# coderforlife/ms-compress

Hardware: AMD Instinct MI355X
Metric: input MB/s (lznt1 compress, bit-exact with the reference CPU encoder) (higher is better)
Workload: dtype u8; 1 GPU; BASELINE configs[4], lznt1: 16x replicated Silesia-shaped set: 192 files, one unit each (4 KiB chunks inside), 3391017280 B; units=192, bytes_rank0=3391017280, parallelism=shard-per-gpu x1, no data-path collective, lznt1_parity_checked=True

## Files before the change

ms_compress_amd/csrc/lznt1.hip:

```cpp
#include "common.h"
#include "kernels.h"

namespace msc {

#ifdef LZ_PROFILE
__device__ unsigned long long g_lz_prof[16];
#define LZ_T(i) { const unsigned long long t_ = __builtin_readcyclecounter(); t_acc[i] += t_ - t_prev; t_prev = t_; }
#define LZ_T0   unsigned long long t_prev = __builtin_readcyclecounter(); unsigned long long t_acc[16] = {0};
#define LZ_CNT(i, v) { t_acc[i] += (unsigned long long)(v); }
#define LZ_TEND if (lane == 0) { for (int i_ = 0; i_ < 16; ++i_) { atomicAdd(&g_lz_prof[i_], t_acc[i_]); } }
#else
#define LZ_T(i)
#define LZ_T0
#define LZ_CNT(i, v)
#define LZ_TEND
#endif

#ifdef LZ4_PROFILE_EVENTS
#define LZ4_PROFILE
#endif
#ifdef LZ4_PROFILE
#define LZ4_NSLOT 20
#define LZ4_NEV   (4 * LZ4_NSLOT)
#define LZ4_NPROF (LZ4_NEV + 4)
// ... 8 lines not shown
#define LZ_SELF     4u
#endif

__device__ __forceinline__ uint32_t lz_hash(uint32_t key24) { const uint32_t h = (key24 * 0x9E3779B1u) >> (32 - LZ_TBL_BITS); return h ? h : 1u; }

__device__ __forceinline__ uint32_t lz_shift(uint32_t pos)
{
	uint32_t z; asm("v_ffbh_u32 %0, %1" : "=v"(z) : "v"(pos - 1u));
	return (z - 16u) < 12u ? z - 16u : 12u;
}

__device__ __forceinline__ void     wst16(uint16_t* p, uint32_t v) { __hip_atomic_store(p, (uint16_t)v, __ATOMIC_RELAXED, __HIP_MEMORY_SCOPE_WAVEFRONT); }
__device__ __forceinline__ uint16_t wld16(uint16_t* p) { return __hip_atomic_load(p, __ATOMIC_RELAXED, __HIP_MEMORY_SCOPE_WAVEFRONT); }
__device__ __forceinline__ void     wst32(uint32_t* p, uint32_t v) { __hip_atomic_store(p, v, __ATOMIC_RELAXED, __HIP_MEMORY_SCOPE_WAVEFRONT); }
__device__ __forceinline__ uint32_t wld32(uint32_t* p) { return __hip_atomic_load(p, __ATOMIC_RELAXED, __HIP_MEMORY_SCOPE_WAVEFRONT); }
__device__ __forceinline__ void     wave_fence() { __builtin_amdgcn_fence(__ATOMIC_ACQ_REL, "wavefront", "local"); }

typedef uint16_t lz_u16x2 __attribute__((ext_vector_type(2)));
__device__ __forceinline__ uint32_t lz_entry32(uint16_t e) { lz_u16x2 v; v.x = e; return __builtin_bit_cast(uint32_t, v); }
__device__ __forceinline__ u64 lz_entry_below(uint32_t e, uint32_t p)
{
	u64 m; asm("v_cmp_gt_u32_sdwa %0, %1, %2 src0_sel:DWORD src1_sel:WORD_0" : "=s"(m) : "v"(p), "v"(e)); return m;
}
__device__ __forceinline__ uint4 lz_ld128(const uint8_t* base, uint32_t off)
{
	const uint32_t* a = reinterpret_cast<const uint32_t*>(base + (off & 0xFFCu));
	const uint32_t w0 = a[0], w1 = a[1], w2 = a[2], w3 = a[3], w4 = a[4];
	return make_uint4(alignbyte_addr(w1, w0, off), alignbyte_addr(w2, w1, off), alignbyte_addr(w3, w2, off), alignbyte_addr(w4, w3, off));
}
__device__ __forceinline__ uint32_t lz_ld32(const uint8_t* base, uint32_t off)
{
	const uint32_t* a = reinterpret_cast<const uint32_t*>(base + (off & 0xFFCu));
	return alignbyte_addr(a[1], a[0], off);
}
__device__ __forceinline__ uint32_t lz_lcp_tail(const uint8_t* d, uint32_t q, uint32_t p, uint32_t maxlen, uint32_t& it)
{
	uint32_t l = 16u;
	for (;;) {
		++it;
		uint4 a, b;
		a = lz_ld128(d, q + l); b = lz_ld128(d, p + l);
		const uint32_t f = first_nz_byte16(a.x ^ b.x, a.y ^ b.y, a.z ^ b.z, a.w ^ b.w);
		l += f;
		if (f < 16u || l >= maxlen) { break; }
	}
	return l;
}
__device__ __forceinline__ uint32_t lz_lcp_wave(const uint8_t* d, uint32_t q, uint32_t p, uint32_t l, uint32_t maxlen, uint32_t lane, uint32_t& steps)
{
	const uint32_t shq = q + l, shp = p + l;
	for (;;) {
		const uint32_t oq = q + l + 4u * lane, op = p + l + 4u * lane;
		const uint32_t* const aq = reinterpret_cast<const uint32_t*>(d + (oq & 0xFFCu));
		const uint32_t* const ap = reinterpret_cast<const uint32_t*>(d + (op & 0xFFCu));
		const uint32_t x = alignbyte_addr(aq[1], aq[0], shq) ^ alignbyte_addr(ap[1], ap[0], shp);
		const u64 ne = __builtin_amdgcn_ballot_w64(x != 0u);
		++steps;
		if (ne) {
			const uint32_t i = ctz64(ne);
			l += 4u * i + ((uint32_t)__builtin_ctz((uint32_t)__builtin_amdgcn_readlane((int)x, (int)i)) >> 3);
			break;
		}
		l += 256u;
		if (l >= maxlen) { break; }
	}
	return l < maxlen ? l : maxlen;
// ... 3 lines not shown
	const uint32_t a = ffbl_raw(x1) | 32u, b = ffbl_raw(x2) | 64u, c = ffbl_raw(x3) | 96u;
	return min3u(min3u(ffbl_raw(x0), a, b), c, capbits);
}
#define LZ_S1 8u
struct LzS1 { uint32_t x, y; };
__device__ __forceinline__ LzS1 lz_ld_s1(const uint8_t* base, uint32_t off)
{
	const uint32_t* a = reinterpret_cast<const uint32_t*>(base + (off & 0xFFCu));
	const uint32_t w0 = a[0], w1 = a[1], w2 = a[2];
	return LzS1{ alignbyte_addr(w1, w0, off), alignbyte_addr(w2, w1, off) };
}
__device__ __forceinline__ uint32_t lz_diff_bits_s1(uint32_t x0, uint32_t x1, uint32_t capbits)
{
	return min3u(ffbl_raw(x0), ffbl_raw(x1) | 32u, capbits);
}
struct LzS2 { uint32_t z, w; };
__device__ __forceinline__ LzS2 lz_ld_s2(const uint8_t* base, uint32_t off)
{
	const uint32_t* a = reinterpret_cast<const uint32_t*>(base + (off & 0xFFCu));
	const uint32_t w2 = a[2], w3 = a[3], w4 = a[4];
	return LzS2{ alignbyte_addr(w3, w2, off), alignbyte_addr(w4, w3, off) };
}
__device__ __forceinline__ uint32_t lz_diff_bits_s2(uint32_t xz, uint32_t xw, uint32_t capbits)
{
	return min3u(ffbl_raw(xz) | 64u, ffbl_raw(xw) | 96u, capbits);
}
__device__ __forceinline__ uint32_t lz_key(uint32_t bits, uint32_t q)
{
	uint32_t r; asm("v_bitop3_b32 %0, %1, %2, %3 bitop3:0x74" : "=v"(r) : "v"(bits << 9), "s"(0xFFFu), "v"(q)); return r;
}
__device__ __forceinline__ uint32_t lz_bit64(u64 m, uint32_t i) { u64 t; asm("s_lshr_b64 %0, %1, %2" : "=s"(t) : "s"(m), "s"(i) : "scc"); return (uint32_t)t & 1u; }
__device__ __forceinline__ uint32_t lz_need_bits(uint32_t len) { uint32_t r; asm("s_lshl3_add_u32 %0, %1, 8" : "=s"(r) : "s"(len) : "scc"); return r; }
struct LzWin { uint32_t key, o0, shift; u64 tokmask, matchmask; };
template <bool packed>
__device__ __forceinline__ uint32_t lz_window(const uint8_t* s_data, const void* tbl, const uint16_t* s_bucket, uint32_t n, uint32_t lane,
                                              uint32_t wbase, uint32_t entry, LzWin& r)
{
	entry = (uint32_t)__builtin_amdgcn_readfirstlane((int)entry); wbase = (uint32_t)__builtin_amdgcn_readfirstlane((int)wbase);
	const uint32_t wend = (wbase + 64u < n) ? wbase + 64u : n;
	const uint32_t p = wbase + lane;
	const LzS1 own = lz_ld_s1(s_data, p);
	const uint32_t o0 = own.x, o1 = own.y;
	const uint32_t shift = lz_shift(p);
	const uint32_t mask3 = (1u << shift) + 2u;
	uint32_t rel;
	asm("s_max_u32 %0, %1, %2\n\ts_sub_u32 %0, %0, %2" : "=&s"(rel) : "s"(entry), "s"(wbase) : "scc");
	const uint32_t lo = (wbase == 0 && rel == 0) ? 1u : rel;
	const uint32_t hi = n > wbase + 2u ? (n - wbase - 2u < 64u ? n - wbase - 2u : 64u) : 0u;
	const u64 act = sgpr64((~(u64)0 << lo) & (hi >= 64u ? ~(u64)0 : (((u64)1 << hi) - 1u)));
	const uint32_t maxlen = (n - p < mask3) ? n - p : mask3;
	uint32_t s;
	{
		const uint32_t h = lz_hash(o0 & 0xFFFFFFu);
		if (packed) {
			const uint32_t bit = h * 12u - 12u;
			const uint32_t* const t = static_cast<const uint32_t*>(tbl) + (bit >> 5);
			s = __builtin_amdgcn_alignbit(t[1], t[0], bit) & 0xFFFu;
		} else {
			s = static_cast<const uint16_t*>(tbl)[h - 1u];
		}
	}
	uint32_t key = 0;
	uint32_t q[LZ_SELF + 1u];
	u64 ex[LZ_SELF + 1u];
	#pragma unroll
	for (uint32_t j = 0; j <= LZ_SELF; ++j) { q[j] = lz_entry32(wld16(const_cast<uint16_t*>(s_bucket) + s + j)); }
	#pragma unroll
	for (uint32_t j = 0; j <= LZ_SELF; ++j) { ex[j] = (j ? ex[j - 1u] : act) & lz_entry_below(q[j], p); }
	const uint32_t capb = (maxlen < 16u ? maxlen : 16u) << 3, cap1 = (maxlen < LZ_S1 ? maxlen : LZ_S1) << 3;
	uint32_t kk[LZ_SELF];
	{
		uint32_t lb[LZ_SELF];
		{
			LzS1 c[LZ_SELF];
			#pragma unroll
			for (uint32_t k = 0; k < LZ_SELF; ++k) { c[k] = lz_ld_s1(s_data, q[k]); }
			#pragma unroll
			for (uint32_t k = 0; k < LZ_SELF; ++k) { lb[k] = lz_diff_bits_s1(c[k].x ^ o0, c[k].y ^ o1, cap1); }
		}
		u64 more = 0;
		#pragma unroll
		for (uint32_t k = 0; k < LZ_SELF; ++k) { more |= __builtin_amdgcn_ballot_w64(lb[k] >= 8u * LZ_S1) & ex[k]; }
		if (more & __builtin_amdgcn_ballot_w64(maxlen > LZ_S1)) {
			const LzS2 a = lz_ld_s2(s_data, p);
			LzS2 c[LZ_SELF];
			#pragma unroll
			for (uint32_t k = 0; k < LZ_SELF; ++k) { c[k] = lz_ld_s2(s_data, q[k]); }
			#pragma unroll
			for (uint32_t k = 0; k < LZ_SELF; ++k) {
				const uint32_t l2 = lz_diff_bits_s2(c[k].z ^ a.z, c[k].w ^ a.w, capb);
				lb[k] = lb[k] >= 8u * LZ_S1 ? l2 : lb[k];
			}
		}
		#pragma unroll
		for (uint32_t k = 0; k < LZ_SELF; ++k) {
			asm("v_cndmask_b32 %0, 0, %1, %2" : "=v"(kk[k]) : "v"(lz_key(lb[k], q[k])), "s"(ex[k]));
			key = kk[k] > key ? kk[k] : key;
		}
	}
	const u64 five = ex[LZ_SELF];
	u64 un = five & __builtin_amdgcn_ballot_w64(key < (maxlen << 12));
	const u64 lp = sgpr64(__builtin_amdgcn_ballot_w64(key >= (16u << 12)) & __builtin_amdgcn_ballot_w64(maxlen > 16u));
	u64 mm = __builtin_amdgcn_ballot_w64(key >= (3u << 12)) & ~un;
	u64 matchmask = 0;
	const uint32_t wn = (uint32_t)__builtin_amdgcn_readfirstlane((int)(wend - wbase));
	un = sgpr64(un); mm = sgpr64(mm);
	const u64 pend = sgpr64(un | lp);
	const uint32_t nx = lane + (key >> 12);
	const u64 restl = (un | mm) >> (nx & 63u);
	const uint32_t zl = min3u(ffbl_raw((uint32_t)restl), ffbl_raw((uint32_t)(restl >> 32)) | 32u, 64u);
	const uint32_t J = (nx + zl < wn) ? nx + zl : wn;
	uint32_t mp;
	{
		u64 rest; asm("s_lshr_b64 %0, %1, %2" : "=s"(rest) : "s"(un | mm), "s"(rel) : "scc");
		mp = rest ? rel + ctz64(rest) : wn;
	}
	if (mp < wn) do {
		asm volatile(
			"s_nop 3\n\t"
			"1:\n\t"
			"s_bitcmp1_b64 %[pend], %[mp]\n\t"
			"s_cbranch_scc1 3f\n\t"
			"s_bitset1_b64 %[mk], %[mp]\n\t"
			"v_readlane_b32 %[mp], %[J], %[mp]\n\t"
			"s_cmp_lt_u32 %[mp], %[wn]\n\t"
			"s_cbranch_scc1 1b\n\t"
			"3:\n\t"
			: [mp] "+s"(mp), [mk] "+s"(matchmask)
			: [pend] "s"(pend), [wn] "s"(wn), [J] "v"(J)
			: "scc");
		if (mp < wn) {
			const uint32_t sL = (uint32_t)__builtin_amdgcn_readlane((int)s, (int)mp);
			const uint32_t maxL = (uint32_t)__builtin_amdgcn_readlane((int)maxlen, (int)mp);
			const uint32_t pL = wbase + mp;
			uint32_t kbest = (uint32_t)__builtin_amdgcn_readlane((int)key, (int)mp);
			uint32_t fin = 1u;
			if (lz_bit64(lp, mp)) {
				const uint32_t qv = s_bucket[sL + lane % LZ_SELF];
				uint32_t nst = 0;
				#pragma unroll
				for (uint32_t k = 0; k < LZ_SELF; ++k) {
					if ((uint32_t)__builtin_amdgcn_readlane((int)kk[k], (int)mp) >> 16) {
						const uint32_t qk = (uint32_t)__builtin_amdgcn_readlane((int)qv, (int)k);
						const uint32_t l = lz_lcp_wave(s_data, qk, pL, 16u, maxL, lane, nst);
						const uint32_t kk = (l << 12) | (qk ^ 4095u);
						kbest = kk > kbest ? kk : kbest;
						if (l == maxL) { break; }
					}
				}
				fin = kbest < (maxL << 12) ? lz_bit64(un, mp) : 0u;
#ifdef LZ4_PROFILE_EVENTS
				if (lane == 0) { atomicAdd(&g_lz4_prof[LZ4_NEV + 2], 1ull); atomicAdd(&g_lz4_prof[LZ4_NEV + 3], (unsigned long long)nst); }
#endif
			}
			asm volatile("" : "+s"(fin));
			if (fin) {
				const uint32_t a0 = (uint32_t)__builtin_amdgcn_readlane((int)o0, (int)mp), a1 = (uint32_t)__builtin_amdgcn_readlane((int)o1, (int)mp);
#ifdef LZ4_PROFILE_EVENTS
				uint32_t nsteps = 0, ntail = 0;
#endif
				const uint32_t cap1L = (maxL < LZ_S1 ? maxL : LZ_S1) << 3;
				uint32_t need = kbest >> 12; need = lz_need_bits(need > 2u ? need : 2u);
				uint32_t base = sL + LZ_SELF;
// ... 31 lines not shown
				if (lane == 0) { atomicAdd(&g_lz4_prof[LZ4_NEV], (unsigned long long)nsteps); atomicAdd(&g_lz4_prof[LZ4_NEV + 1], (unsigned long long)ntail); }
#endif
			}
			{
				uint32_t t; u64 rs;
#pragma clang diagnostic push
#pragma clang diagnostic ignored "-Winline-asm"
				asm volatile(
					"s_bitset0_b64 %[un], %[mp]\n\t"
					"s_mov_b32 m0, %[mp]\n\t"
					"s_lshr_b32 %[t], %[kb], 12\n\t"
					"s_cmp_gt_u32 %[t], 2\n\t"
					"s_cselect_b32 %[t], %[t], 1\n\t"
					"s_cbranch_scc0 5f\n\t"
					"s_bitset1_b64 %[mk], %[mp]\n\t"
					"5:\n\t"
					"v_writelane_b32 %[key], %[kb], m0\n\t"
					"s_add_u32 %[mp], %[mp], %[t]\n\t"
					"s_or_b64 %[rs], %[un], %[mm]\n\t"
					"s_lshr_b64 %[rs], %[rs], %[mp]\n\t"
					"s_ff1_i32_b64 %[t], %[rs]\n\t"
					"s_min_u32 %[t], %[t], 64\n\t"
					"s_add_u32 %[mp], %[mp], %[t]\n\t"
					: [un] "+s"(un), [mk] "+s"(matchmask), [mp] "+s"(mp), [key] "+v"(key), [t] "=&s"(t), [rs] "=&s"(rs)
					: [kb] "s"(kbest), [mm] "s"(mm)
					: "scc", "m0");
#pragma clang diagnostic pop
			}
		}
	} while (mp < wn);
	matchmask = sgpr64(matchmask);
	uint32_t mend; asm("v_cndmask_b32 %0, 0, %1, %2" : "=v"(mend) : "v"(p + (key >> 12)), "s"(matchmask));
	const uint32_t reach = wave_incl_scan_max(mend);
	const u64 range = (~(u64)0 << rel) & (wn >= 64u ? ~(u64)0 : (((u64)1 << wn) - 1u));
	const u64 tokmask = range & (matchmask | __builtin_amdgcn_ballot_w64(reach <= p));
	const uint32_t wreach = (uint32_t)__builtin_amdgcn_readlane((int)reach, 63);
	const uint32_t cur = wreach > wend ? wreach : wend;

	r.key = key; r.o0 = o0; r.shift = shift; r.tokmask = tokmask; r.matchmask = matchmask;
	return cur;
}

template <bool serial>
__device__ __forceinline__ uint32_t lz_ordered_add(uint32_t* addr, uint32_t v, bool active, uint32_t lane)
{
	uint32_t old = 0;
	if (!serial) { if (active) { old = __hip_atomic_fetch_add(addr, v, __ATOMIC_RELAXED, __HIP_MEMORY_SCOPE_WAVEFRONT); } }
	else { for (uint32_t l = 0; l < 64u; ++l) { if (lane == l && active) { old = __hip_atomic_fetch_add(addr, v, __ATOMIC_RELAXED, __HIP_MEMORY_SCOPE_WAVEFRONT); } wave_fence(); } }
	return old;
}

template <bool serial, bool DEV = false>
__global__ __launch_bounds__(64) void lznt1_chunk_kernel(const uint8_t* __restrict__ d_in, BatchTables bt,
                                                        uint8_t* __restrict__ slots, uint32_t* __restrict__ slot_size)
{
	struct __attribute__((aligned(16))) Lds {
		uint8_t  data[4096 + 32];
		uint16_t bucket[4096];
		uint16_t cnt[LZ_TBL];
		uint32_t flagacc[16];
		uint32_t flagpos[16];
	};
	__shared__ Lds L;
	uint8_t* const s_data = L.data; uint16_t* const s_cnt = L.cnt; uint16_t* const s_bucket = L.bucket;
	uint32_t* const s_flagacc = L.flagacc; uint32_t* const s_flagpos = L.flagpos;

	const uint32_t lane = threadIdx.x;
// ... 134 lines not shown
extern "C" void mscomp_amd_debug_lz_prof(unsigned long long* out, int reset)
{
	(void)hipMemcpyFromSymbol(out, HIP_SYMBOL(g_lz_prof), sizeof(unsigned long long) * 16);
	if (reset) { unsigned long long z[16] = {0}; (void)hipMemcpyToSymbol(HIP_SYMBOL(g_lz_prof), z, sizeof z); }
}
#endif

#define LZ4_NSEG 4u
#ifndef LZ4_B1
#define LZ4_B1 21u
#define LZ4_B2 38u
#define LZ4_B3 52u
#endif
__device__ __forceinline__ uint32_t lz4_seg_start(uint32_t j) { return j == 0 ? 0u : j == 1 ? LZ4_B1 : j == 2 ? LZ4_B2 : j == 3 ? LZ4_B3 : 64u; }
#ifndef LZ4_P1
#define LZ4_P1 15u
#define LZ4_P2 39u
#endif
__host__ __device__ constexpr uint32_t lz4_max3(uint32_t a, uint32_t b, uint32_t c) { return a > b ? (a > c ? a : c) : (b > c ? b : c); }
__host__ __device__ constexpr uint32_t lz4_field_bits(uint32_t batches) { return batches * 64u <= 0x3FFu ? 10u : 11u; }
#define LZ4_PMAX lz4_max3(LZ4_P1, LZ4_P2 - LZ4_P1, 64u - LZ4_P2)
#define LZ4_F0 lz4_field_bits(LZ4_P1)
#define LZ4_F1 lz4_field_bits(LZ4_P2 - LZ4_P1)
#define LZ4_F2 lz4_field_bits(64u - LZ4_P2)
static_assert(LZ4_P1 >= 1u && LZ4_P1 < LZ4_P2 && LZ4_P2 < 64u, "three parts, none empty");
static_assert(LZ4_P1 * 64u <= (1u << LZ4_F0) - 1u && (LZ4_P2 - LZ4_P1) * 64u <= (1u << LZ4_F1) - 1u && (64u - LZ4_P2) * 64u <= (1u << LZ4_F2) - 1u, "a part fits its count field");
static_assert(LZ4_F0 + LZ4_F1 + LZ4_F2 <= 32u, "the three fields share a dword");
static_assert(LZ4_P1 <= LZ4_PMAX && LZ4_P2 - LZ4_P1 <= LZ4_PMAX && 64u - LZ4_P2 <= LZ4_PMAX, "LZ4_PMAX");
#define LZ4_MAXM 22u
#ifdef LZ4_PROFILE
extern "C" void mscomp_amd_debug_lz4_prof(unsigned long long* out) { (void)hipMemcpyFromSymbol(out, HIP_SYMBOL(g_lz4_prof), sizeof(unsigned long long) * LZ4_NPROF); unsigned long long z[LZ4_NPROF] = {0}; (void)hipMemcpyToSymbol(HIP_SYMBOL(g_lz4_prof), z, sizeof z); }
#endif
static_assert(LZNT1_REC == 2u * 64u * LZ4_MAXM * sizeof(uint16_t), "kernels.h: LZNT1_REC = two areas of 64 windows of match tokens");
template <bool serial, bool DEV = false>
__global__ __launch_bounds__(256) void lznt1_chunk4_kernel(const uint8_t* __restrict__ d_in, BatchTables bt,
                                                          uint8_t* __restrict__ slots, uint32_t* __restrict__ slot_size, uint16_t* __restrict__ recs)
{
	struct Ctl {
		u64      tok[64], mat[64];
		uint16_t endc[64];
		uint32_t prog[LZ4_NSEG];
		uint32_t used[LZ4_NSEG];
		uint32_t segctr;
		uint32_t total[2];
		uint8_t  rep[64];
	};
	struct __attribute__((aligned(16))) Lds {
		uint8_t  data[4096];
		uint16_t bucket[4096];
		union {
			uint16_t cnt[LZ_TBL];
			struct { uint32_t ends[LZ_TBL * 12u / 32u]; Ctl ctl; } parse;
		} t;
	};
	static_assert(LZ_TBL == 4096u, "the pack below hands 16 bucket ends to each of 256 threads");
	static_assert(sizeof(Lds) <= 20480, "eight blocks per CU");
	static_assert(offsetof(Lds, t) == offsetof(Lds, bucket) + sizeof(Lds::bucket) && sizeof(Lds::bucket) + sizeof(Lds::t) == LZ_TBL * sizeof(uint32_t),
	              "the sort's count words (one dword per bucket) lie over the bucket array and the union behind it");
	__shared__ Lds L;
	uint32_t* const s_cw = reinterpret_cast<uint32_t*>(L.bucket);
	uint8_t* const s_data = L.data; uint16_t* const s_cnt = L.t.cnt; uint16_t* const s_bucket = L.bucket;
	Ctl& C = L.t.parse.ctl;
	u64* const s_tok = C.tok; u64* const s_mat = C.mat; uint16_t* const s_endc = C.endc; uint8_t* const s_rep = C.rep;
	uint32_t* const s_prog = C.prog; uint32_t* const s_used = C.used; uint32_t& s_segctr = C.segctr; uint32_t* const s_total = C.total;
	uint16_t* const s_T = s_cnt;
	uint16_t* const s_S = s_cnt + 64;
	uint16_t* const s_flagpos = s_cnt + 128;
	uint32_t* const s_flagacc = reinterpret_cast<uint32_t*>(s_cnt + 640);

	const uint32_t tid = threadIdx.x, lane = tid & 63u;
	uint32_t c, wv;
	c = blockIdx.x; wv = (uint32_t)__builtin_amdgcn_readfirstlane((int)(tid >> 6));
	if (DEV && past_real_chunks(bt, c)) { if (tid == 0) { slot_size[c] = 0; } return; }
	uint32_t park = 0;
#define LZ4_PARK(i, v) { park = lane == (i) ? (uint32_t)(v) : park; }
#define LZ4_FETCH(i) ({ asm volatile("" : "+v"(park)); (uint32_t)__builtin_amdgcn_readlane((int)park, (int)(i)); })
	LZ4_PARK(0, (uintptr_t)slots) LZ4_PARK(1, (uintptr_t)slots >> 32) LZ4_PARK(2, (uintptr_t)slot_size) LZ4_PARK(3, (uintptr_t)slot_size >> 32)
	LZ4_PARK(4, c) LZ4_PARK(5, wv)
	asm volatile("" : "+v"(park));
	const uint32_t u = unit_of_chunk(bt.chunk_prefix, bt.n_units, c);
	const u64 coff = (u64)(c - bt.chunk_prefix[u]) * 4096u;
	const u64 left = bt.in_len[u] - coff;
	const uint32_t n = left < 4096u ? (uint32_t)left : 4096u;
	const uint8_t* __restrict__ src = d_in + bt.in_off[u] + coff;
	uint16_t* __restrict__ rec = recs + (u64)c * (LZNT1_REC / sizeof(uint16_t));

#ifdef LZ4_PROFILE
	uint32_t z_prev; asm volatile("v_mov_b32 %0, %1" : "=v"(z_prev) : "s"((uint32_t)__builtin_readcyclecounter()));
	uint32_t z_acc = 0;
#define LZ4_T(i) { uint32_t t_; asm volatile("v_mov_b32 %0, %1" : "=v"(t_) : "s"((uint32_t)__builtin_readcyclecounter())); z_acc += lane == (i) ? t_ - z_prev : 0u; z_prev = t_; }
#define LZ4_TEND { if (lane < LZ4_NSLOT) { atomicAdd(&g_lz4_prof[LZ4_NSLOT * wv + lane], (unsigned long long)z_acc); } }
#else
#define LZ4_T(i)
#define LZ4_TEND
#endif
	{
		const uint32_t nvec = (((uintptr_t)src & 15u) == 0) ? (n & ~15u) : 0u;
		for (uint32_t i = tid * 16u; i < nvec; i += 4096u) { *reinterpret_cast<uint4*>(s_data + i) = *reinterpret_cast<const uint4*>(src + i); }
		for (uint32_t i = nvec + tid; i < n; i += 256u) { s_data[i] = src[i]; }
		for (uint32_t i = n + tid; i < 4096u; i += 256u) { s_data[i] = 0; }
		for (uint32_t i = tid * 4u; i < LZ_TBL; i += 1024u) { *reinterpret_cast<uint4*>(s_cw + i) = make_uint4(0, 0, 0, 0); }
	}
	LZ4_T(0)
	__syncthreads();
	LZ4_T(1)
	{
		const uint32_t nb = (n + 63u) >> 6;
		const uint32_t pb0 = wv == 0 ? 0u : wv == 1u ? LZ4_P1 : wv == 2u ? LZ4_P2 : 64u;
		const uint32_t pe = wv == 0 ? LZ4_P1 : wv == 1u ? LZ4_P2 : 64u;
		const uint32_t pb1 = pe < nb ? pe : nb;
		const uint32_t fsh = wv == 0 ? 0u : wv == 1u ? LZ4_F0 : LZ4_F0 + LZ4_F1;
		const uint32_t fm = (1u << (wv == 0 ? LZ4_F0 : wv == 1u ? LZ4_F1 : LZ4_F2)) - 1u;
		uint32_t hr[LZ4_PMAX];
		#pragma unroll
		for (uint32_t i = 0; i < LZ4_PMAX; ++i) { hr[i] = 0; }
		#pragma unroll
		for (uint32_t j0 = 0; j0 < LZ4_PMAX; j0 += 8u) {
			if (pb0 + j0 < pb1) {
				uint32_t h[8], old[8];
				#pragma unroll
				for (uint32_t j = 0; j < 8u; ++j) { if (j0 + j < LZ4_PMAX) { h[j] = lz_hash(lz_ld32(s_data, (pb0 + j0 + j) * 64u + lane) & 0xFFFFFFu); } }
				#pragma unroll
				for (uint32_t j = 0; j < 8u; ++j) {
					if (j0 + j < LZ4_PMAX) { const uint32_t b = pb0 + j0 + j; old[j] = lz_ordered_add<serial>(s_cw + h[j], 1u << fsh, b < pb1 && b * 64u + lane + 2u < n, lane); }
				}
				#pragma unroll
				for (uint32_t j = 0; j < 8u; ++j) { if (j0 + j < LZ4_PMAX) { hr[j0 + j] = (h[j] << 12) | ((old[j] >> fsh) & fm); } }
			}
		}
		LZ4_T(2)
		__syncthreads();
		LZ4_T(3)
		static_assert(LZ4_P2 * 64u < 4096u, "rank + counts in front stay in 12 bits");
		if (wv == 1u || wv == 2u) {
			const uint32_t m1 = wv == 2u ? (1u << LZ4_F1) - 1u : 0u;
			#pragma unroll
			for (uint32_t j0 = 0; j0 < LZ4_PMAX; j0 += 8u) {
				if (pb0 + j0 < pb1) {
					uint32_t w[8];
					#pragma unroll
					for (uint32_t j = 0; j < 8u; ++j) { if (j0 + j < LZ4_PMAX) { w[j] = s_cw[hr[j0 + j] >> 12]; } }
					#pragma unroll
					for (uint32_t j = 0; j < 8u; ++j) { if (j0 + j < LZ4_PMAX) { hr[j0 + j] += (w[j] & ((1u << LZ4_F0) - 1u)) + ((w[j] >> LZ4_F0) & m1); } }
					__builtin_amdgcn_sched_barrier(0);
				}
			}
		}
		uint32_t tot[8], sum = 0;
		#pragma unroll
		for (uint32_t k = 0; k < 4u; ++k) {
			const uint4 a = reinterpret_cast<const uint4*>(s_cw)[4u * tid + k];
			uint32_t x[4] = { a.x, a.y, a.z, a.w };
			#pragma unroll
			for (uint32_t i = 0; i < 4u; ++i) { x[i] = (x[i] & ((1u << LZ4_F0) - 1u)) + ((x[i] >> LZ4_F0) & ((1u << LZ4_F1) - 1u)) + (x[i] >> (LZ4_F0 + LZ4_F1)); }
			if (k == 0 && tid == 0) { x[0] = 0; }
			sum += (x[0] + x[1]) + (x[2] + x[3]);
			tot[2u * k] = x[0] | (x[1] << 16); tot[2u * k + 1u] = x[2] | (x[3] << 16);
// ... 13 lines not shown
			uint32_t* const o = L.t.parse.ends + 6u * tid;
			#pragma unroll
			for (int k = 0; k < 2; ++k) {
				uint32_t v[8];
				#pragma unroll
				for (int i = 0; i < 4; ++i) { r += tot[4 * k + i] & 0xFFFFu; v[2 * i] = r; r += tot[4 * k + i] >> 16; v[2 * i + 1] = r; }
				o[3 * k]      = v[0] | (v[1] << 12) | (v[2] << 24);
				o[3 * k + 1u] = (v[2] >> 8) | (v[3] << 4) | (v[4] << 16) | (v[5] << 28);
				o[3 * k + 2u] = (v[5] >> 4) | (v[6] << 8) | (v[7] << 20);
			}
			if (tid < LZ4_NSEG) { s_prog[tid] = 0; s_used[tid] = 0; }
			if (tid < 16u) { reinterpret_cast<uint32_t*>(s_rep)[tid] = 0; }
			if (tid == 0) { s_segctr = 0; }
		}
		LZ4_T(6)
		__syncthreads();
		LZ4_T(7)
		#pragma unroll
		for (uint32_t j0 = 0; j0 < LZ4_PMAX; j0 += 8u) {
			if (pb0 + j0 < pb1) {
				uint32_t st[8];
				#pragma unroll
				for (uint32_t j = 0; j < 8u; ++j) {
					if (j0 + j < LZ4_PMAX) {
						const uint32_t bit = (hr[j0 + j] >> 12) * 12u - 12u;
						const uint32_t* const t = L.t.parse.ends + (bit >> 5);
						st[j] = __builtin_amdgcn_alignbit(t[1], t[0], bit) & 0xFFFu;
					}
				}
				#pragma unroll
				for (uint32_t j = 0; j < 8u; ++j) {
					if (j0 + j < LZ4_PMAX) {
						const uint32_t b = pb0 + j0 + j, p = b * 64u + lane;
						if (b < pb1 && p + 2u < n) { s_bucket[st[j] + (hr[j0 + j] & 0xFFFu)] = (uint16_t)p; }
					}
				}
			}
		}
	}
	LZ4_T(8)
	__syncthreads();
	const uint32_t* const tbl = L.t.parse.ends;
	LZ4_T(9)

	const uint32_t nw = (n + 63u) >> 6;
#define LZ4_WINDOW(w_, entry_, cur_out, a_) { \
		const uint32_t wb_ = (w_) * 64u; const uint32_t we_ = (wb_ + 64u < n) ? wb_ + 64u : n; \
		if ((entry_) >= we_) { if (lane == 0) { s_tok[w_] = 0; s_mat[w_] = 0; } cur_out = (entry_); } \
		else { \
			LzWin r_; cur_out = lz_window<true>(s_data, tbl, s_bucket, n, lane, wb_, (entry_), r_); \
			if (__builtin_amdgcn_inverse_ballot_w64(r_.matchmask)) { \
				const uint32_t p_ = wb_ + lane, best_ = r_.key >> 12; \
				uint16_t* __restrict__ const recw_ = rec + ((a_) * 64u + (w_)) * LZ4_MAXM; \
				recw_[popc_below(r_.matchmask)] = (uint16_t)(((p_ - (4095u - (r_.key & 0xFFFu)) - 1u) << r_.shift) | (best_ - 3u)); \
			} \
			if (lane == 0) { s_tok[w_] = r_.tokmask; s_mat[w_] = r_.matchmask; } \
		} \
		if ((a_) && lane == 0) { s_rep[w_] = 1; } }
#define LZ4_UNI(x) ((uint32_t)__builtin_amdgcn_readfirstlane((int)(x)))
	for (;;) {
		uint32_t seg = 0;
		if (lane == 0) { seg = atomicAdd(&s_segctr, 1u); }
		seg = (uint32_t)__builtin_amdgcn_readfirstlane((int)seg);
		const uint32_t a0 = lz4_seg_start(seg);
		if (a0 >= nw) { break; }
		const uint32_t a1 = (lz4_seg_start(seg + 1u) < nw) ? lz4_seg_start(seg + 1u) : nw;
		uint32_t entry = a0 * 64u;
		for (uint32_t w = a0; w < a1; w = LZ4_UNI(w + 1u)) {
			uint32_t cur;
			LZ4_WINDOW(w, entry, cur, 0u)
			entry = LZ4_UNI(cur);
			if (lane == 0) { s_endc[w] = (uint16_t)cur; }
			wave_fence();
			if (lane == 0) { __hip_atomic_store(&s_prog[seg], w + 1u, __ATOMIC_RELAXED, __HIP_MEMORY_SCOPE_WORKGROUP); }
		}
		if (a1 < nw) {
			if (lane == 0) { s_used[seg + 1u] = entry; }
			if (entry != a1 * 64u) {
				const uint32_t wlim = (lz4_seg_start(seg + 2u) < nw) ? lz4_seg_start(seg + 2u) : nw;
				for (uint32_t w = a1; w < wlim; w = LZ4_UNI(w + 1u)) {
					while (LZ4_UNI(__hip_atomic_load(&s_prog[seg + 1u], __ATOMIC_RELAXED, __HIP_MEMORY_SCOPE_WORKGROUP)) <= w) { __builtin_amdgcn_s_sleep(2); }
					wave_fence();
					const uint32_t spec = LZ4_UNI(s_endc[w]);
					uint32_t cur;
					LZ4_WINDOW(w, entry, cur, 1u)
					entry = LZ4_UNI(cur);
// ... 13 lines not shown
			if (e2 == LZ4_UNI(s_used[j])) { continue; }
			uint32_t wl = lz4_seg_start(j);
			for (uint32_t w = lz4_seg_start(j); w < nw; w = LZ4_UNI(w + 1u)) {
				const uint32_t spec = LZ4_UNI(s_endc[w]);
				uint32_t cur;
				LZ4_WINDOW(w, e2, cur, 1u)
				e2 = LZ4_UNI(cur);
				if (lane == 0) { s_endc[w] = (uint16_t)cur; }
				wave_fence();
				wl = w + 1u;
				if (cur == spec) { break; }
			}
			if (lane == 0) { for (uint32_t jj = j + 1u; jj < LZ4_NSEG && lz4_seg_start(jj) < wl; ++jj) { s_used[jj] = s_endc[lz4_seg_start(jj) - 1u]; } }
			wave_fence();
		}
	}
	LZ4_T(12)
	__syncthreads();
	LZ4_T(13)
	for (uint32_t i = tid; i < 512u; i += 256u) { s_flagacc[i] = 0; }
	wv = LZ4_FETCH(5); c = LZ4_FETCH(4);
	const uint32_t w0 = wv * 16u, w1 = (w0 + 16u < nw) ? w0 + 16u : nw;
	typedef __attribute__((address_space(1))) uint8_t  g_u8;
	typedef __attribute__((address_space(1))) uint32_t g_u32;
	g_u8* __restrict__ const img = (g_u8*)((uintptr_t)LZ4_FETCH(0) | ((uintptr_t)LZ4_FETCH(1) << 32)) + (u64)c * LZNT1_SLOT;
	g_u32* __restrict__ const szp = (g_u32*)((uintptr_t)LZ4_FETCH(2) | ((uintptr_t)LZ4_FETCH(3) << 32)) + c;
	static_assert(LZNT1_SLOT <= 0xFFFFFFFFu && (LZ4_MAXM & 1u) == 0 && LZ4_NSEG * 16u * LZ4_MAXM <= 4096u, "a window's tokens are whole dwords; four pieces fit the bucket array");
	uint32_t* const s_ptk = reinterpret_cast<uint32_t*>(s_bucket) + wv * (16u * LZ4_MAXM / 2u);
	const uint32_t wl0 = w0 + (lane & 15u);
	const u64 tokv = wl0 < w1 ? s_tok[wl0] : (u64)0, matv = wl0 < w1 ? s_mat[wl0] : (u64)0;
#ifndef LZ4_PROBE_EMIT
	{
		const uint32_t info = wl0 < w1 ? (uint32_t)__popcll(matv) | ((uint32_t)s_rep[wl0] << 8) : 0u;
		const uint32_t* __restrict__ const rec32 = reinterpret_cast<const uint32_t*>(rec);
		uint32_t v[3]; bool ld[3];
		#pragma unroll
		for (uint32_t k = 0; k < 3u; ++k) {
			const uint32_t idx = lane + 64u * k, wl = idx / (LZ4_MAXM / 2u), m2 = idx - wl * (LZ4_MAXM / 2u);
			const uint32_t inf = (uint32_t)__builtin_amdgcn_ds_bpermute((int)(wl * 4u), (int)info);
			ld[k] = idx < 16u * LZ4_MAXM / 2u && 2u * m2 < (inf & 0xFFu);
			v[k] = ld[k] ? rec32[((inf >> 8) * 64u + w0 + wl) * (LZ4_MAXM / 2u) + m2] : 0u;
		}
		#pragma unroll
		for (uint32_t k = 0; k < 3u; ++k) { if (ld[k]) { s_ptk[lane + 64u * k] = v[k]; } }
	}
#endif
	if (wv == 0) {
		const u64 tm = lane < nw ? s_tok[lane] : (u64)0, mk = lane < nw ? s_mat[lane] : (u64)0;
		const uint32_t nt = (uint32_t)__popcll(tm), ns = nt + (uint32_t)__popcll(mk);
		const uint32_t ti = wave_incl_scan_add_u32(nt), si = wave_incl_scan_add_u32(ns);
		s_T[lane] = (uint16_t)(ti - nt); s_S[lane] = (uint16_t)(si - ns);
		if (lane == 63u) { s_total[0] = ti; s_total[1] = si; }
	}
	LZ4_T(14)
	__syncthreads();
	LZ4_T(15)
	const uint32_t T = s_total[0], S = s_total[1];
	const uint32_t csize = ((T + 7u) >> 3) + S;
	uint32_t total;
	if (csize < n) {
		const uint32_t tsv = (uint32_t)s_T[wl0] | ((uint32_t)s_S[wl0] << 16);
		const uint32_t nwin = LZ4_UNI(w1 > w0 ? w1 - w0 : 0u);
		#pragma unroll 1
		for (uint32_t k = 0; k < nwin; ++k) {
			const u64 tokmask = ((u64)(uint32_t)__builtin_amdgcn_readlane((int)(uint32_t)(tokv >> 32), (int)k) << 32) | (uint32_t)__builtin_amdgcn_readlane((int)(uint32_t)tokv, (int)k);
			if (tokmask == 0) { continue; }
			const u64 matchmask = ((u64)(uint32_t)__builtin_amdgcn_readlane((int)(uint32_t)(matv >> 32), (int)k) << 32) | (uint32_t)__builtin_amdgcn_readlane((int)(uint32_t)matv, (int)k);
// ... 6 lines not shown
				const uint32_t lit = s_data[(w0 + k) * 64u + lane];
#ifdef LZ4_PROBE_EMIT
				const uint16_t tok = 0x1003u;
#else
				const uint16_t tok = reinterpret_cast<const uint16_t*>(s_ptk)[k * LZ4_MAXM + mbl];
#endif
				uint32_t lo; asm("v_cndmask_b32 %0, %1, %2, %3" : "=v"(lo) : "v"(lit), "v"(lz_entry32(tok)), "s"(matchmask));
				img[pos] = (uint8_t)lo;
				if (__builtin_amdgcn_inverse_ballot_w64(matchmask)) {
					uint32_t p1 = pos; asm("" : "+v"(p1));
					(img + p1)[1] = (uint8_t)(tok >> 8);
					atomicOr(&s_flagacc[t >> 3], 1u << (t & 7u));
				}
			}
		}
		LZ4_T(16)
		__syncthreads();
		LZ4_T(17)
		#pragma unroll 1
		for (uint32_t g = tid; g < ((T + 7u) >> 3); g += 256u) { uint32_t fp = s_flagpos[g]; asm("" : "+v"(fp)); img[fp] = (uint8_t)s_flagacc[g]; }
		if (tid == 0) { img[0] = (uint8_t)(0xB000u | (csize - 1u)); img[1] = (uint8_t)((0xB000u | (csize - 1u)) >> 8); }
		total = 2u + csize;
	} else {
		const uint32_t hdr = 0x3000u | (n - 1u);
		for (uint32_t k = tid; k < (n + 2u + 3u) / 4u; k += 256u) {
			uint32_t o = 4u * k; asm("" : "+v"(o));
			*(g_u32*)(img + o) = (k == 0) ? (hdr | (ld16(s_data) << 16)) : ld32(s_data + 4u * k - 2u);
		}
		total = 2u + n;
	}
	if (tid == 0) { *szp = total; }
	LZ4_T(18)
	LZ4_TEND
#undef LZ4_WINDOW
#undef LZ4_UNI
#undef LZ4_PARK
#undef LZ4_FETCH
}

template <bool DEV>
static void launch_lznt1_chunks_t(hipStream_t st, const uint8_t* d_in, const BatchTables& bt, uint8_t* slots, uint32_t* slot_size, uint16_t* recs,
                                  int mode, bool serial)
{
	if (mode == 1) {
		if (serial) { hipLaunchKernelGGL((lznt1_chunk_kernel<true, DEV>), dim3(bt.n_chunks), dim3(64), 0, st, d_in, bt, slots, slot_size); }
		else { hipLaunchKernelGGL((lznt1_chunk_kernel<false, DEV>), dim3(bt.n_chunks), dim3(64), 0, st, d_in, bt, slots, slot_size); }
	} else {
		if (serial) { hipLaunchKernelGGL((lznt1_chunk4_kernel<true, DEV>), dim3(bt.n_chunks), dim3(256), 0, st, d_in, bt, slots, slot_size, recs); }
		else { hipLaunchKernelGGL((lznt1_chunk4_kernel<false, DEV>), dim3(bt.n_chunks), dim3(256), 0, st, d_in, bt, slots, slot_size, recs); }
	}
}
void launch_lznt1_chunks_dev(hipStream_t st, const uint8_t* d_in, const BatchTables& bt, uint8_t* slots, uint32_t* slot_size, uint16_t* recs,
                             int mode, bool serial);
#ifndef LZNT1_DEV_TU
static int g_lznt1_mode = 0;
void set_lznt1_mode(int mode) { g_lznt1_mode = mode; }
void launch_lznt1_chunks(hipStream_t st, const uint8_t* d_in, const BatchTables& bt, uint8_t* slots, uint32_t* slot_size, uint16_t* recs, bool dev)
{
	if (bt.n_chunks == 0) { return; }
	const int mode = g_lznt1_mode ? g_lznt1_mode : 2;
	const bool serial = serial_atomics_on_current_device();
	if (dev) { launch_lznt1_chunks_dev(st, d_in, bt, slots, slot_size, recs, mode, serial); }
	else { launch_lznt1_chunks_t<false>(st, d_in, bt, slots, slot_size, recs, mode, serial); }
}
#else
void launch_lznt1_chunks_dev(hipStream_t st, const uint8_t* d_in, const BatchTables& bt, uint8_t* slots, uint32_t* slot_size, uint16_t* recs,
                             int mode, bool serial)
{
// ... 6 lines not shown
```

Measured before the change: 88850 MB/s.

## Specialize LZNT1 chunk kernel body for full 4 KiB chunks

Splits the chunk4 kernel into a templated body that is instantiated twice, once for full 4096-byte chunks and once for any length, and picks between them at runtime. In the full-chunk version, window bounds, active masks, the walk-loop limit and the hash-insert predicates become compile-time constants, and a lane-based aligned load replaces the general unaligned load. The aim is to cut scalar bookkeeping and branches in the hot window loop for nearly all chunks. In exchange the code is larger, which risks instruction-cache pressure and higher register use.

```diff
diff --git a/ms_compress_amd/csrc/lznt1.hip b/ms_compress_amd/csrc/lznt1.hip
--- a/ms_compress_amd/csrc/lznt1.hip
+++ b/ms_compress_amd/csrc/lznt1.hip
@@ -64,6 +64,11 @@
 {
 	const uint32_t* a = reinterpret_cast<const uint32_t*>(base + (off & 0xFFCu));
 	return alignbyte_addr(a[1], a[0], off);
+}
+__device__ __forceinline__ uint32_t lz_ld32_lane(const uint8_t* a4, uint32_t lane)
+{
+	const uint32_t* a = reinterpret_cast<const uint32_t*>(a4);
+	return alignbyte_addr(a[1], a[0], lane);
 }
 __device__ __forceinline__ uint32_t lz_lcp_tail(const uint8_t* d, uint32_t q, uint32_t p, uint32_t maxlen, uint32_t& it)
 {
@@ -133,12 +138,13 @@
 __device__ __forceinline__ uint32_t lz_bit64(u64 m, uint32_t i) { u64 t; asm("s_lshr_b64 %0, %1, %2" : "=s"(t) : "s"(m), "s"(i) : "scc"); return (uint32_t)t & 1u; }
 __device__ __forceinline__ uint32_t lz_need_bits(uint32_t len) { uint32_t r; asm("s_lshl3_add_u32 %0, %1, 8" : "=s"(r) : "s"(len) : "scc"); return r; }
 struct LzWin { uint32_t key, o0, shift; u64 tokmask, matchmask; };
-template <bool packed>
+template <bool packed, bool FULL = false>
 __device__ __forceinline__ uint32_t lz_window(const uint8_t* s_data, const void* tbl, const uint16_t* s_bucket, uint32_t n, uint32_t lane,
                                               uint32_t wbase, uint32_t entry, LzWin& r)
 {
+	if (FULL) { n = 4096u; }
 	entry = (uint32_t)__builtin_amdgcn_readfirstlane((int)entry); wbase = (uint32_t)__builtin_amdgcn_readfirstlane((int)wbase);
-	const uint32_t wend = (wbase + 64u < n) ? wbase + 64u : n;
+	const uint32_t wend = FULL ? wbase + 64u : ((wbase + 64u < n) ? wbase + 64u : n);
 	const uint32_t p = wbase + lane;
 	const LzS1 own = lz_ld_s1(s_data, p);
 	const uint32_t o0 = own.x, o1 = own.y;
@@ -146,9 +152,18 @@
 	const uint32_t mask3 = (1u << shift) + 2u;
 	uint32_t rel;
 	asm("s_max_u32 %0, %1, %2\n\ts_sub_u32 %0, %0, %2" : "=&s"(rel) : "s"(entry), "s"(wbase) : "scc");
-	const uint32_t lo = (wbase == 0 && rel == 0) ? 1u : rel;
-	const uint32_t hi = n > wbase + 2u ? (n - wbase - 2u < 64u ? n - wbase - 2u : 64u) : 0u;
-	const u64 act = sgpr64((~(u64)0 << lo) & (hi >= 64u ? ~(u64)0 : (((u64)1 << hi) - 1u)));
+	u64 act;
+	if (FULL) {
+		uint32_t lo;
+		asm("s_or_b32 %0, %1, %2\n\ts_cselect_b32 %0, %2, 1" : "=&s"(lo) : "s"(wbase), "s"(rel) : "scc");
+		const uint32_t top = wbase == 4032u ? 0x3FFFFFFFu : 0xFFFFFFFFu;
+		const u64 m = ~(u64)0 << lo;
+		act = sgpr64(((u64)((uint32_t)(m >> 32) & top) << 32) | (uint32_t)m);
+	} else {
+		const uint32_t lo = (wbase == 0 && rel == 0) ? 1u : rel;
+		const uint32_t hi = n > wbase + 2u ? (n - wbase - 2u < 64u ? n - wbase - 2u : 64u) : 0u;
+		act = sgpr64((~(u64)0 << lo) & (hi >= 64u ? ~(u64)0 : (((u64)1 << hi) - 1u)));
+	}
 	const uint32_t maxlen = (n - p < mask3) ? n - p : mask3;
 	uint32_t s;
 	{
@@ -204,7 +219,7 @@
 	const u64 lp = sgpr64(__builtin_amdgcn_ballot_w64(key >= (16u << 12)) & __builtin_amdgcn_ballot_w64(maxlen > 16u));
 	u64 mm = __builtin_amdgcn_ballot_w64(key >= (3u << 12)) & ~un;
 	u64 matchmask = 0;
-	const uint32_t wn = (uint32_t)__builtin_amdgcn_readfirstlane((int)(wend - wbase));
+	const uint32_t wn = FULL ? 64u : (uint32_t)__builtin_amdgcn_readfirstlane((int)(wend - wbase));
 	un = sgpr64(un); mm = sgpr64(mm);
 	const u64 pend = sgpr64(un | lp);
 	const uint32_t nx = lane + (key >> 12);
@@ -217,19 +232,22 @@
 		mp = rest ? rel + ctz64(rest) : wn;
 	}
 	if (mp < wn) do {
-		asm volatile(
-			"s_nop 3\n\t"
-			"1:\n\t"
-			"s_bitcmp1_b64 %[pend], %[mp]\n\t"
-			"s_cbranch_scc1 3f\n\t"
-			"s_bitset1_b64 %[mk], %[mp]\n\t"
-			"v_readlane_b32 %[mp], %[J], %[mp]\n\t"
-			"s_cmp_lt_u32 %[mp], %[wn]\n\t"
-			"s_cbranch_scc1 1b\n\t"
+#define LZ_WALK(WN_) \
+			"s_nop 3\n\t" \
+			"1:\n\t" \
+			"s_bitcmp1_b64 %[pend], %[mp]\n\t" \
+			"s_cbranch_scc1 3f\n\t" \
+			"s_bitset1_b64 %[mk], %[mp]\n\t" \
+			"v_readlane_b32 %[mp], %[J], %[mp]\n\t" \
+			"s_cmp_lt_u32 %[mp], " WN_ "\n\t" \
+			"s_cbranch_scc1 1b\n\t" \
 			"3:\n\t"
-			: [mp] "+s"(mp), [mk] "+s"(matchmask)
-			: [pend] "s"(pend), [wn] "s"(wn), [J] "v"(J)
-			: "scc");
+		if (FULL) {
+			asm volatile(LZ_WALK("64") : [mp] "+s"(mp), [mk] "+s"(matchmask) : [pend] "s"(pend), [J] "v"(J) : "scc");
+		} else {
+			asm volatile(LZ_WALK("%[wn]") : [mp] "+s"(mp), [mk] "+s"(matchmask) : [pend] "s"(pend), [wn] "s"(wn), [J] "v"(J) : "scc");
+		}
+#undef LZ_WALK
 		if (mp < wn) {
 			const uint32_t sL = (uint32_t)__builtin_amdgcn_readlane((int)s, (int)mp);
 			const uint32_t maxL = (uint32_t)__builtin_amdgcn_readlane((int)maxlen, (int)mp);
@@ -327,7 +345,7 @@
 	matchmask = sgpr64(matchmask);
 	uint32_t mend; asm("v_cndmask_b32 %0, 0, %1, %2" : "=v"(mend) : "v"(p + (key >> 12)), "s"(matchmask));
 	const uint32_t reach = wave_incl_scan_max(mend);
-	const u64 range = (~(u64)0 << rel) & (wn >= 64u ? ~(u64)0 : (((u64)1 << wn) - 1u));
+	const u64 range = FULL ? ~(u64)0 << rel : (~(u64)0 << rel) & (wn >= 64u ? ~(u64)0 : (((u64)1 << wn) - 1u));
 	const u64 tokmask = range & (matchmask | __builtin_amdgcn_ballot_w64(reach <= p));
 	const uint32_t wreach = (uint32_t)__builtin_amdgcn_readlane((int)reach, 63);
 	const uint32_t cur = wreach > wend ? wreach : wend;
@@ -528,32 +546,50 @@
 extern "C" void mscomp_amd_debug_lz4_prof(unsigned long long* out) { (void)hipMemcpyFromSymbol(out, HIP_SYMBOL(g_lz4_prof), sizeof(unsigned long long) * LZ4_NPROF); unsigned long long z[LZ4_NPROF] = {0}; (void)hipMemcpyToSymbol(HIP_SYMBOL(g_lz4_prof), z, sizeof z); }
 #endif
 static_assert(LZNT1_REC == 2u * 64u * LZ4_MAXM * sizeof(uint16_t), "kernels.h: LZNT1_REC = two areas of 64 windows of match tokens");
-template <bool serial, bool DEV = false>
-__global__ __launch_bounds__(256) void lznt1_chunk4_kernel(const uint8_t* __restrict__ d_in, BatchTables bt,
-                                                          uint8_t* __restrict__ slots, uint32_t* __restrict__ slot_size, uint16_t* __restrict__ recs)
-{
-	struct Ctl {
-		u64      tok[64], mat[64];
-		uint16_t endc[64];
-		uint32_t prog[LZ4_NSEG];
-		uint32_t used[LZ4_NSEG];
-		uint32_t segctr;
-		uint32_t total[2];
-		uint8_t  rep[64];
-	};
-	struct __attribute__((aligned(16))) Lds {
-		uint8_t  data[4096];
-		uint16_t bucket[4096];
-		union {
-			uint16_t cnt[LZ_TBL];
-			struct { uint32_t ends[LZ_TBL * 12u / 32u]; Ctl ctl; } parse;
-		} t;
-	};
-	static_assert(LZ_TBL == 4096u, "the pack below hands 16 bucket ends to each of 256 threads");
-	static_assert(sizeof(Lds) <= 20480, "eight blocks per CU");
-	static_assert(offsetof(Lds, t) == offsetof(Lds, bucket) + sizeof(Lds::bucket) && sizeof(Lds::bucket) + sizeof(Lds::t) == LZ_TBL * sizeof(uint32_t),
-	              "the sort's count words (one dword per bucket) lie over the bucket array and the union behind it");
-	__shared__ Lds L;
+struct Lz4Ctl {
+	u64      tok[64], mat[64];
+	uint16_t endc[64];
+	uint32_t prog[LZ4_NSEG];
+	uint32_t used[LZ4_NSEG];
+	uint32_t segctr;
+	uint32_t total[2];
+	uint8_t  rep[64];
+};
+struct __attribute__((aligned(16))) Lz4Lds {
+	uint8_t  data[4096];
+	uint16_t bucket[4096];
+	union {
+		uint16_t cnt[LZ_TBL];
+		struct { uint32_t ends[LZ_TBL * 12u / 32u]; Lz4Ctl ctl; } parse;
+	} t;
+};
+static_assert(LZ_TBL == 4096u, "the pack below hands 16 bucket ends to each of 256 threads");
+static_assert(sizeof(Lz4Lds) <= 20480, "eight blocks per CU");
+static_assert(offsetof(Lz4Lds, t) == offsetof(Lz4Lds, bucket) + sizeof(Lz4Lds::bucket) && sizeof(Lz4Lds::bucket) + sizeof(Lz4Lds::t) == LZ_TBL * sizeof(uint32_t),
+              "the sort's count words (one dword per bucket) lie over the bucket array and the union behind it");
+#define LZ4_PARK(i, v) { park = lane == (i) ? (uint32_t)(v) : park; }
+#define LZ4_FETCH(i) ({ asm volatile("" : "+v"(park)); (uint32_t)__builtin_amdgcn_readlane((int)park, (int)(i)); })
+__host__ __device__ constexpr bool lz4_slot_sure(uint32_t i)
+{
+	const uint32_t j0 = i & ~7u, l0 = LZ4_P1, l1 = LZ4_P2 - LZ4_P1, l2 = 64u - LZ4_P2;
+	return !(l0 > j0 && l0 <= i) && !(l1 > j0 && l1 <= i) && !(l2 > j0 && l2 <= i);
+}
+#define LZ4_LAST_SLOT (64u - LZ4_P2 - 1u)
+template <bool serial, bool DEV, bool FULL>
+__device__ __forceinline__ void lz4_chunk_body(Lz4Lds& L, uint32_t park, const uint32_t tid, const uint32_t lane, uint32_t wv)
+{
+	typedef __attribute__((address_space(1))) const uint8_t  gc_u8;
+	typedef uint32_t u32x4 __attribute__((ext_vector_type(4)));
+	typedef __attribute__((address_space(1))) const u32x4    gc_u4;
+	typedef __attribute__((address_space(1))) const uint32_t gc_u32;
+	typedef __attribute__((address_space(1))) uint16_t       g_u16;
+	gc_u8* __restrict__ const src = (gc_u8*)((uintptr_t)LZ4_FETCH(6) | ((uintptr_t)LZ4_FETCH(7) << 32));
+	g_u16* __restrict__ const rec = (g_u16*)((uintptr_t)LZ4_FETCH(8) | ((uintptr_t)LZ4_FETCH(9) << 32));
+	const uint32_t n = FULL ? 4096u : LZ4_FETCH(10);
+#define LZ4_BODY_EDGE(what) { if (FULL) { asm volatile("; lznt1 full-chunk body " what); } else { asm volatile("; lznt1 any-length body " what); } }
+	LZ4_BODY_EDGE("begins")
+	typedef Lz4Ctl Ctl;
+	uint32_t c;
 	uint32_t* const s_cw = reinterpret_cast<uint32_t*>(L.bucket);
 	uint8_t* const s_data = L.data; uint16_t* const s_cnt = L.t.cnt; uint16_t* const s_bucket = L.bucket;
 	Ctl& C = L.t.parse.ctl;
@@ -564,22 +600,6 @@
 	uint16_t* const s_flagpos = s_cnt + 128;
 	uint32_t* const s_flagacc = reinterpret_cast<uint32_t*>(s_cnt + 640);
 
-	const uint32_t tid = threadIdx.x, lane = tid & 63u;
-	uint32_t c, wv;
-	c = blockIdx.x; wv = (uint32_t)__builtin_amdgcn_readfirstlane((int)(tid >> 6));
-	if (DEV && past_real_chunks(bt, c)) { if (tid == 0) { slot_size[c] = 0; } return; }
-	uint32_t park = 0;
-#define LZ4_PARK(i, v) { park = lane == (i) ? (uint32_t)(v) : park; }
-#define LZ4_FETCH(i) ({ asm volatile("" : "+v"(park)); (uint32_t)__builtin_amdgcn_readlane((int)park, (int)(i)); })
-	LZ4_PARK(0, (uintptr_t)slots) LZ4_PARK(1, (uintptr_t)slots >> 32) LZ4_PARK(2, (uintptr_t)slot_size) LZ4_PARK(3, (uintptr_t)slot_size >> 32)
-	LZ4_PARK(4, c) LZ4_PARK(5, wv)
-	asm volatile("" : "+v"(park));
-	const uint32_t u = unit_of_chunk(bt.chunk_prefix, bt.n_units, c);
-	const u64 coff = (u64)(c - bt.chunk_prefix[u]) * 4096u;
-	const u64 left = bt.in_len[u] - coff;
-	const uint32_t n = left < 4096u ? (uint32_t)left : 4096u;
-	const uint8_t* __restrict__ src = d_in + bt.in_off[u] + coff;
-	uint16_t* __restrict__ rec = recs + (u64)c * (LZNT1_REC / sizeof(uint16_t));
 
 #ifdef LZ4_PROFILE
 	uint32_t z_prev; asm volatile("v_mov_b32 %0, %1" : "=v"(z_prev) : "s"((uint32_t)__builtin_readcyclecounter()));
@@ -592,7 +612,7 @@
 #endif
 	{
 		const uint32_t nvec = (((uintptr_t)src & 15u) == 0) ? (n & ~15u) : 0u;
-		for (uint32_t i = tid * 16u; i < nvec; i += 4096u) { *reinterpret_cast<uint4*>(s_data + i) = *reinterpret_cast<const uint4*>(src + i); }
+		for (uint32_t i = tid * 16u; i < nvec; i += 4096u) { *reinterpret_cast<u32x4*>(s_data + i) = *(gc_u4*)(src + i); }
 		for (uint32_t i = nvec + tid; i < n; i += 256u) { s_data[i] = src[i]; }
 		for (uint32_t i = n + tid; i < 4096u; i += 256u) { s_data[i] = 0; }
 		for (uint32_t i = tid * 4u; i < LZ_TBL; i += 1024u) { *reinterpret_cast<uint4*>(s_cw + i) = make_uint4(0, 0, 0, 0); }
@@ -610,15 +630,22 @@
 		uint32_t hr[LZ4_PMAX];
 		#pragma unroll
 		for (uint32_t i = 0; i < LZ4_PMAX; ++i) { hr[i] = 0; }
+		uint32_t inc = 1u << fsh;
+		if (FULL) { asm("v_mov_b32 %0, %1" : "=v"(inc) : "s"(1u << fsh)); }
 		#pragma unroll
 		for (uint32_t j0 = 0; j0 < LZ4_PMAX; j0 += 8u) {
 			if (pb0 + j0 < pb1) {
 				uint32_t h[8], old[8];
 				#pragma unroll
-				for (uint32_t j = 0; j < 8u; ++j) { if (j0 + j < LZ4_PMAX) { h[j] = lz_hash(lz_ld32(s_data, (pb0 + j0 + j) * 64u + lane) & 0xFFFFFFu); } }
+				for (uint32_t j = 0; j < 8u; ++j) { if (j0 + j < LZ4_PMAX) { h[j] = lz_hash(lz_ld32_lane(s_data + (pb0 + j0) * 64u + (lane & 0x3Cu) + 64u * j, lane) & 0xFFFFFFu); } }
 				#pragma unroll
 				for (uint32_t j = 0; j < 8u; ++j) {
-					if (j0 + j < LZ4_PMAX) { const uint32_t b = pb0 + j0 + j; old[j] = lz_ordered_add<serial>(s_cw + h[j], 1u << fsh, b < pb1 && b * 64u + lane + 2u < n, lane); }
+					if (j0 + j < LZ4_PMAX) {
+						const uint32_t b = pb0 + j0 + j;
+						const bool act = FULL ? (lz4_slot_sure(j0 + j) || b < pb1) && (j0 + j != LZ4_LAST_SLOT || b * 64u + lane + 2u < n)
+						                      : b < pb1 && b * 64u + lane + 2u < n;
+						old[j] = lz_ordered_add<serial>(s_cw + h[j], inc, act, lane);
+					}
 				}
 				#pragma unroll
 				for (uint32_t j = 0; j < 8u; ++j) { if (j0 + j < LZ4_PMAX) { hr[j0 + j] = (h[j] << 12) | ((old[j] >> fsh) & fm); } }
@@ -698,7 +725,9 @@
 				for (uint32_t j = 0; j < 8u; ++j) {
 					if (j0 + j < LZ4_PMAX) {
 						const uint32_t b = pb0 + j0 + j, p = b * 64u + lane;
-						if (b < pb1 && p + 2u < n) { s_bucket[st[j] + (hr[j0 + j] & 0xFFFu)] = (uint16_t)p; }
+						const bool act = FULL ? (lz4_slot_sure(j0 + j) || b < pb1) && (j0 + j != LZ4_LAST_SLOT || p + 2u < n)
+						                      : b < pb1 && p + 2u < n;
+						if (act) { s_bucket[st[j] + (hr[j0 + j] & 0xFFFu)] = (uint16_t)p; }
 					}
 				}
 			}
@@ -711,13 +740,13 @@
 
 	const uint32_t nw = (n + 63u) >> 6;
 #define LZ4_WINDOW(w_, entry_, cur_out, a_) { \
-		const uint32_t wb_ = (w_) * 64u; const uint32_t we_ = (wb_ + 64u < n) ? wb_ + 64u : n; \
+		const uint32_t wb_ = (w_) * 64u; const uint32_t we_ = FULL ? wb_ + 64u : ((wb_ + 64u < n) ? wb_ + 64u : n); \
 		if ((entry_) >= we_) { if (lane == 0) { s_tok[w_] = 0; s_mat[w_] = 0; } cur_out = (entry_); } \
 		else { \
-			LzWin r_; cur_out = lz_window<true>(s_data, tbl, s_bucket, n, lane, wb_, (entry_), r_); \
+			LzWin r_; cur_out = lz_window<true, FULL>(s_data, tbl, s_bucket, n, lane, wb_, (entry_), r_); \
 			if (__builtin_amdgcn_inverse_ballot_w64(r_.matchmask)) { \
 				const uint32_t p_ = wb_ + lane, best_ = r_.key >> 12; \
-				uint16_t* __restrict__ const recw_ = rec + ((a_) * 64u + (w_)) * LZ4_MAXM; \
+				g_u16* __restrict__ const recw_ = rec + ((a_) * 64u + (w_)) * LZ4_MAXM; \
 				recw_[popc_below(r_.matchmask)] = (uint16_t)(((p_ - (4095u - (r_.key & 0xFFFu)) - 1u) << r_.shift) | (best_ - 3u)); \
 			} \
 			if (lane == 0) { s_tok[w_] = r_.tokmask; s_mat[w_] = r_.matchmask; } \
@@ -797,7 +826,7 @@
 #ifndef LZ4_PROBE_EMIT
 	{
 		const uint32_t info = wl0 < w1 ? (uint32_t)__popcll(matv) | ((uint32_t)s_rep[wl0] << 8) : 0u;
-		const uint32_t* __restrict__ const rec32 = reinterpret_cast<const uint32_t*>(rec);
+		gc_u32* __restrict__ const rec32 = (gc_u32*)rec;
 		uint32_t v[3]; bool ld[3];
 		#pragma unroll
 		for (uint32_t k = 0; k < 3u; ++k) {
@@ -870,8 +899,33 @@
 	if (tid == 0) { *szp = total; }
 	LZ4_T(18)
 	LZ4_TEND
+	LZ4_BODY_EDGE("ends")
+#undef LZ4_BODY_EDGE
 #undef LZ4_WINDOW
 #undef LZ4_UNI
+}
+
+template <bool serial, bool DEV = false>
+__global__ __launch_bounds__(256) void lznt1_chunk4_kernel(const uint8_t* __restrict__ d_in, BatchTables bt,
+                                                          uint8_t* __restrict__ slots, uint32_t* __restrict__ slot_size, uint16_t* __restrict__ recs)
+{
+	__shared__ Lz4Lds L;
+	const uint32_t tid = threadIdx.x, lane = tid & 63u;
+	const uint32_t c = blockIdx.x, wv = (uint32_t)__builtin_amdgcn_readfirstlane((int)(tid >> 6));
+	if (DEV && past_real_chunks(bt, c)) { if (tid == 0) { slot_size[c] = 0; } return; }
+	uint32_t park = 0;
+	LZ4_PARK(0, (uintptr_t)slots) LZ4_PARK(1, (uintptr_t)slots >> 32) LZ4_PARK(2, (uintptr_t)slot_size) LZ4_PARK(3, (uintptr_t)slot_size >> 32)
+	LZ4_PARK(4, c) LZ4_PARK(5, wv)
+	const uint32_t u = unit_of_chunk(bt.chunk_prefix, bt.n_units, c);
+	const u64 coff = (u64)(c - bt.chunk_prefix[u]) * 4096u;
+	const u64 left = bt.in_len[u] - coff;
+	const uint32_t n = left < 4096u ? (uint32_t)left : 4096u;
+	const uint8_t* __restrict__ src = d_in + bt.in_off[u] + coff;
+	uint16_t* __restrict__ rec = recs + (u64)c * (LZNT1_REC / sizeof(uint16_t));
+	LZ4_PARK(6, (uintptr_t)src) LZ4_PARK(7, (uintptr_t)src >> 32) LZ4_PARK(8, (uintptr_t)rec) LZ4_PARK(9, (uintptr_t)rec >> 32) LZ4_PARK(10, n)
+	asm volatile("" : "+v"(park));
+	if ((uint32_t)__builtin_amdgcn_readfirstlane((int)n) == 4096u) { lz4_chunk_body<serial, DEV, true>(L, park, tid, lane, wv); }
+	else { lz4_chunk_body<serial, DEV, false>(L, park, tid, lane, wv); }
 #undef LZ4_PARK
 #undef LZ4_FETCH
 }
```

Result: faster. 92910 MB/s, median of 6 (+4.6%).
